# arneschneuing/DiffSBDD

Hardware: AMD Instinct MI355X
Metric: sampled ligands/sec (500-step DDPM, fullatom_cond) at 1/2/4/8 MI355X (higher is better)
Workload: dtype f32

## Files before the change

diffsbdd_amd/_lib.py:

```python
from __future__ import annotations

import ctypes as C
import os

_HERE = os.path.dirname(os.path.abspath(__file__))
LIB_PATH = os.environ.get("DSBDD_LIB") or os.path.join(_HERE, "libdiffsbdd_hip.so")
ABI_VERSION = 6

OK, ERR_ARG, ERR_STATE, ERR_CAPACITY, ERR_LAUNCH = 0, -1, -2, -3, -4
STATUS_NAN, STATUS_EDGE_OVERFLOW = 1, 2
MOL_MAX_ATOMS, MOL_STATS, FP_WORDS = 128, 8, 64

G_NAMES = ["ATOM_ENC_W0T", "ATOM_ENC_B0", "ATOM_ENC_W1T", "ATOM_ENC_B1",
           "RES_ENC_W0T", "RES_ENC_B0", "RES_ENC_W1T", "RES_ENC_B1",
           "ATOM_DEC_W0T", "ATOM_DEC_B0", "ATOM_DEC_W1T", "ATOM_DEC_B1",
           "RES_DEC_W0T", "RES_DEC_B0", "RES_DEC_W1T", "RES_DEC_B1",
           "EMB_WT", "EMB_B", "EMBOUT_WT", "EMBOUT_B"]
GCL_NAMES = ["E1_WT", "E1_WD", "E1_WD0", "E1_TAB", "E2_WT", "E2_B", "ATT_W", "ATT_B",
             "N1_WT", "N1_B", "N2_WT", "N2_B"]
EQ_NAMES = ["C1_WT", "C_WD", "C_WD0", "C_TAB", "C_W2T", "C_B2",
            "X_WD", "X_WD0", "X_TAB", "X_W2T", "X_B2", "W3"]
OPT_PRUNE, OPT_CONE, OPT_GRANULE16, OPT_EMU, OPT_SPLITK, OPT_SHELL, OPT_TAIL = 0, 1, 2, 3, 4, 5, 6
(BUF_EDGE_ROW, BUF_EDGE_COL, BUF_EDGE_D0, BUF_ROW_PTR, BUF_H, BUF_X, BUF_NODE_BATCH, BUF_DEG,
 BUF_LEVEL, BUF_LEVEL_LIST, BUF_LEVEL_COUNT, BUF_LEVEL_END, BUF_LROW_PTR, BUF_LEDGE_ROW, BUF_LEDGE_COL,
 BUF_LEDGE_D0, BUF_LEVEL_STATS) = range(17)


class Config(C.Structure):
    _fields_ = [(n, C.c_int32) for n in (
        "atom_nf", "residue_nf", "joint_nf", "hidden_nf", "n_layers", "inv_sublayers",
        "attention", "use_tanh", "update_pocket_coords", "reflection_equivariant",
        "edge_embedding_dim", "has_cutoff_ligand", "has_cutoff_pocket",
        "has_cutoff_interaction")] + [(n, C.c_float) for n in (
            "cutoff_ligand", "cutoff_pocket", "cutoff_interaction",
            "norm_constant", "normalization_factor", "coords_range")]


class TrainGraph(C.Structure):
    _fields_ = [(n, C.c_void_p) for n in ("erow", "ecol", "ed0", "row_ptr", "deg", "rev", "node_batch", "lig_off",
                                          "poc_off")] + [(n, C.c_int64) for n in ("n_lig", "n_nodes", "n_edges", "batch")]


class LossCfg(C.Structure):
    _fields_ = [(n, C.c_int32) for n in ("batch", "n_lig", "n_pocket", "atom_nf", "residue_nf", "timesteps", "remove_com",
                                         "vnode_idx")] + \
# ... 43 lines not shown
    "dsbdd_engine_set_option": (C.c_int, [_P, C.c_int, C.c_int]),
    "dsbdd_engine_get_option": (C.c_int, [_P, C.c_int]),
    "dsbdd_engine_profile": (C.c_int, [_P, C.c_int, C.c_int]),
    "dsbdd_engine_profile_read": (C.c_int, [_P, C.POINTER(C.c_double), C.POINTER(_I64)]),
    "dsbdd_cond_reverse_update": (C.c_int, [_P, _P, _P, _P, _P, _P, _P, _I64, _I64, _I64,
                                            _I32, _I32, _F, _F, _F, _I32]),
    "dsbdd_joint_reverse_update": (C.c_int, [_P, _P, _P, _P, _P, _P, _P, _P, _P, _I64, _I64, _I64,
                                             _I32, _I32, _F, _F, _F, _I32]),
    "dsbdd_segment_mean3": (C.c_int, [_P, _P, _I32, _P, _I64, _I64, _P]),
    "dsbdd_cond_affine_noise": (C.c_int, [_P, _P, _P, _P, _P, _P, _I64, _I64, _I64, _I32, _I32, _F, _F, _I32]),
    "dsbdd_joint_affine_noise": (C.c_int, [_P, _P, _P, _P, _P, _P, _P, _I64, _I64, _I64, _I32, _I32, _F, _F,
                                           _I32, _I32]),
    "dsbdd_cond_repaint_update": (C.c_int, [_P, _P, _P, _P, _P, _P, _P, _P, _P, _P, _P, _I64, _I64, _I64,
                                            _I32, _I32, _F, _F, _F, _F, _I32, _I32]),
    "dsbdd_joint_repaint_update": (C.c_int, [_P] * 15 + [_I64, _I64, _I64, _I32, _I32, _F, _F, _F, _F, _I32]),
    "dsbdd_cond_step_keyed": (C.c_int, [_P] * 10 + [_I64, _I64, _I64, _I32, _I32, _F, _F, _F, _I32, _F, _F, _F, _I32,
                                        C.c_uint64, C.c_uint64, _I64, _P, _P, _F]),
    "dsbdd_randn_keyed": (C.c_int, [_P, _P, _P, _I64, _I32, _I64, _I64, _P, C.c_uint64, C.c_uint64,
                                    C.c_uint32]),
    "dsbdd_node_linear": (C.c_int, [_P, _P, _I32, _I32, _P, _I32, _I32, _P, _I32, _P, _P, _I32,
                                    _P, _I32, _I64, _I32, _I32]),
    "dsbdd_chain_split_host": (_I64, [_I32, _I32, _I32, _P, _P, _P, _I32, _I32, _P, _P, _I64]),
    "dsbdd_chain_split_probe": (C.c_int, [_P, _I32, _P, _I32, _I32, _P, _P, _P, _I32, _I32, _P, _P, _I64, _P]),
    "dsbdd_build_edges": (C.c_int, [_P, _P, _P, _P, _I64, _I64, _I64, C.POINTER(Config),
                                    _P, _P, _P, _P, _P, _P, _P, _P, _I64, _P]),
    "dsbdd_bond_orders": (C.c_int, [_P, _P, _P, _P, _I64, _I32, _P, _P, _P, C.c_float, C.c_float,
                                    C.c_float, _I32, _P]),
    "dsbdd_mol_graph_stats": (C.c_int, [_P, _P, _P, _P, _I64, _I32, _P, _I32, _I32, _P, _P, _P, _P, _P, _P]),
    "dsbdd_fp_diversity": (C.c_int, [_P, _P, _P, _I64, _P, _P]),
    "dsbdd_pose_check": (C.c_int, [_P, _P, _P, _P, _I64, _P, _P, _P, _P, _I64, _F, _F, _P, _P]),
    "dsbdd_vina_type": (C.c_int, [_P, _P, _P, _P, _I64, _I32, _P, _I32, _P, _P]),
    "dsbdd_vina_score": (C.c_int, [_P, _P, _P, _P, _I64, _P, _P, _P, _P, _P, _I64, _P, _P, _P]),
    "dsbdd_vina_score_grad": (C.c_int, [_P, _P, _P, _P, _I64, _P, _P, _P, _P, _P, _I64, _P, _P, _P, _P, _P]),
    "dsbdd_vina_minimize": (C.c_int, [_P, _P, _P, _P, _I64, _P, _P, _P, _P, _P, _I64, _P, _P, _P, _P, _P, _F, _F, _I32, _P, _P,
                                      _P, _P]),
    "dsbdd_pack_ligands": (C.c_int, [_P, _P, _P, _P, _I32, _I64, _P, _P, _P, _I64, _I64, _I32, _P, _P, _P, _P, _P]),
    "dsbdd_train_scratch_bytes": (C.c_size_t, [_I32, _I64, _I64]),
    "dsbdd_train_wgrad_scratch_bytes": (C.c_size_t, [_I64, _I64, _I64]),
    "dsbdd_train_wgrad_plan_bytes": (C.c_size_t, [_I64, _I64, _I64]),
    "dsbdd_train_edge_rev": (C.c_int, [_P, _P, _P]),
    "dsbdd_train_sample_mean": (C.c_int, [_P, _P, _P, _P]),
    "dsbdd_train_gcl_forward": (C.c_int, [_P, _I32, _P, _P, _P, _F, _P, _P, C.c_size_t]),
    "dsbdd_train_gcl_backward": (C.c_int, [_P, _I32, _P, _P, _P, _F, _P, _P, _P, _P, C.c_size_t]),
    "dsbdd_train_coord_forward": (C.c_int, [_P, _I32, _P, _P, _I32, _P, _P, _I64, _F, _F, _I32, _F, _P, _P,
                                            C.c_size_t]),
    "dsbdd_train_coord_backward": (C.c_int, [_P, _I32, _P, _P, _I32, _P, _P, _I64, _I64, _F, _F, _I32, _F, _P, _P, _P,
# ... 91 lines not shown
```

diffsbdd_amd/csrc/capi_kernels.h:

```cpp
#pragma once

extern "C" {

int dsbdd_cond_reverse_update(void* stream, float* z_lig, float* xh_pocket, const float* eps_lig,
                              const float* noise, const int64_t* mask_lig, const int64_t* mask_pocket,
                              int64_t n_lig, int64_t n_pocket, int64_t batch, int32_t atom_nf,
                              int32_t residue_nf, float alpha_ts, float c_eps, float sigma, int32_t remove_com) {
  StreamDevice stream_device_(stream);
  if (!z_lig || !xh_pocket || !eps_lig || !noise || !mask_lig || !mask_pocket || batch < 1)
    return fail(DSBDD_ERR_ARG, "bad argument");
  hipLaunchKernelGGL(cond_update_kernel, dim3((int)batch), dim3(kThreads), 0, static_cast<hipStream_t>(stream),
                     z_lig, xh_pocket, eps_lig, noise, mask_lig, (int)n_lig, mask_pocket, (int)n_pocket,
                     3 + atom_nf, 3 + residue_nf, alpha_ts, c_eps, sigma, remove_com);
  HIP_TRY(hipGetLastError());
  return DSBDD_OK;
}

int dsbdd_joint_reverse_update(void* stream, float* z_lig, float* z_pocket, const float* eps_lig,
                               const float* eps_pocket, const float* noise_lig, const float* noise_pocket,
                               const int64_t* mask_lig, const int64_t* mask_pocket, int64_t n_lig,
                               int64_t n_pocket, int64_t batch, int32_t atom_nf, int32_t residue_nf,
                               float alpha_ts, float c_eps, float sigma, int32_t center_noise) {
  StreamDevice stream_device_(stream);
  if (!z_lig || !z_pocket || !eps_lig || !eps_pocket || !noise_lig || !noise_pocket || !mask_lig ||
// ... 122 lines not shown
  HIP_TRY(hipGetLastError());
  return DSBDD_OK;
}

int dsbdd_node_linear(void* stream, const float* A1, int32_t lda1, int32_t K1, const float* A2, int32_t lda2,
                      int32_t K2, const float* WT, int32_t ldw, const float* bias, const float* R, int32_t ldr,
                      float* C, int32_t ldc, int64_t M, int32_t N, int32_t act) {
  StreamDevice stream_device_(stream);
  if (!A1 || !WT || !C || K1 < 1 || K2 < 0 || (K2 > 0 && !A2) || (ldw & 3) || N > ldw ||
      (reinterpret_cast<uintptr_t>(WT) & 15))
    return fail(DSBDD_ERR_ARG, "bad argument (WT must be 16-byte aligned with ldw % 4 == 0)");
  HIP_TRY(nl(static_cast<hipStream_t>(stream), A1, lda1, K1, A2, lda2, K2, WT, ldw, bias, R, ldr, C, ldc, M, N, act));
  return DSBDD_OK;
}

static bool chain_split_args_ok(int32_t M, int32_t n_proj, const void* proj_N, const void* proj_first, const void* proj_count,
                                int32_t H, int32_t grid, const void* header, const void* pieces, int64_t capacity) {
  return header && capacity >= 0 && (capacity == 0 || pieces) && grid >= 1 && (H == 64 || H == 128 || H == 192 || H == 256) &&
         n_proj >= 0 && n_proj <= kChainMaxProj && (n_proj == 0 || (proj_N && proj_first && proj_count)) && M <= (8 << 20);
}
static const char* const kChainSplitBadArg =
    "bad argument (null output, grid < 1, H not 64 / 128 / 192 / 256, more than 3 projections or more than 8 M rows)";

int64_t dsbdd_chain_split_host(int32_t M, int32_t do_mlp, int32_t n_proj, const int32_t* proj_N,
                               const int32_t* proj_first, const int32_t* proj_count, int32_t H, int32_t grid,
                               uint32_t* header, int32_t* pieces, int64_t capacity) {
  if (!chain_split_args_ok(M, n_proj, proj_N, proj_first, proj_count, H, grid, header, pieces, capacity))
    return fail(DSBDD_ERR_ARG, kChainSplitBadArg);
  ChainSplitIn in{};
  in.M = M; in.do_mlp = do_mlp; in.n_proj = n_proj; in.H = H; in.grid = grid;
  for (int q = 0; q < n_proj; ++q) { in.N[q] = proj_N[q]; in.first[q] = proj_first[q]; in.count[q] = proj_count[q]; }
  const ChainSplit sp(in);
  sp.report(header);
  return chain_split_list(sp, grid, grid, ~0u, pieces, capacity);
}

int dsbdd_chain_split_probe(void* stream, int32_t M, const int32_t* m_count, int32_t do_mlp, int32_t n_proj,
                            const int32_t* proj_N, const int32_t* proj_first, const int32_t* const* proj_count,
                            int32_t H, int32_t grid, uint32_t* header, int32_t* pieces, int64_t capacity,
                            int64_t* n_pieces) {
  StreamDevice stream_device_(stream);
  if (!n_pieces || !chain_split_args_ok(M, n_proj, proj_N, proj_first, proj_count, H, grid, header, pieces, capacity))
    return fail(DSBDD_ERR_ARG, kChainSplitBadArg);
  NodeChainArgs a{};
  a.M = M; a.m_count = m_count; a.do_mlp = do_mlp; a.n_proj = n_proj;
  for (int q = 0; q < n_proj; ++q) { a.proj[q].N = proj_N[q]; a.proj[q].first = proj_first[q]; a.proj[q].count = proj_count[q]; }
  hipLaunchKernelGGL(chain_split_probe_kernel, dim3(grid), dim3(64), 0, static_cast<hipStream_t>(stream), a, (int)H, header,
                     pieces, (long long)capacity, reinterpret_cast<long long*>(n_pieces));
  HIP_TRY(hipGetLastError());
  return DSBDD_OK;
}

int dsbdd_bond_orders(void* stream, const float* x, const int32_t* atom_type, const int32_t* mol_off,
                      int64_t batch, int32_t n_types, const float* bonds1, const float* bonds2,
                      const float* bonds3, float margin1, float margin2, float margin3, int32_t n_max,
                      int8_t* order) {
  StreamDevice stream_device_(stream);
  if (!x || !atom_type || !mol_off || !bonds1 || !bonds2 || !bonds3 || !order || batch < 1 || n_types < 1 ||
      n_max < 1)
    return fail(DSBDD_ERR_ARG, "bad argument");
  hipStream_t s = static_cast<hipStream_t>(stream);
  HIP_TRY(hipMemsetAsync(order, 0, (size_t)batch * n_max * n_max, s));
  BondArgs a{x, atom_type, mol_off, bonds1, bonds2, bonds3, margin1, margin2, margin3, n_types, n_max,
             reinterpret_cast<signed char*>(order)};
  hipLaunchKernelGGL(bond_orders_kernel, dim3((unsigned)batch), dim3(64), 0, s, a);
  HIP_TRY(hipGetLastError());
  return DSBDD_OK;
}

int dsbdd_mol_graph_stats(void* stream, const int8_t* order, const int32_t* atom_type, const int32_t* mol_off, int64_t batch,
                          int32_t n_types, const int32_t* max_valence, int32_t n_max, int32_t orders_in_key,
                          int32_t* valence, int32_t* label, int32_t* stats, uint64_t* keys, uint32_t* fingerprint,
                          int32_t* type_counts) {
// ... 165 lines not shown
```

diffsbdd_amd/csrc/chain_split.h:

```cpp
#pragma once

#ifdef __HIPCC__
#define CHAIN_SPLIT_FN __host__ __device__ __forceinline__
#else
#define CHAIN_SPLIT_FN inline
#endif
namespace dsbdd {
constexpr int kChainRowsMax = 96;
constexpr int kChainMaxProj = 3;
constexpr int kChainAllRows = 0x7fffffff;
constexpr int kChainBreaks = 2 * kChainMaxProj + 3;
template <class T> CHAIN_SPLIT_FN T chain_min(T a, T b) { return b < a ? b : a; }
template <class T> CHAIN_SPLIT_FN T chain_max(T a, T b) { return a < b ? b : a; }
CHAIN_SPLIT_FN unsigned chain_share(unsigned a, unsigned j, unsigned n) { return a / n * j + (a % n * j + n - 1) / n; }

struct ChainSplitIn {
  int M;
  int do_mlp, n_proj;
  int N[kChainMaxProj];
  int first[kChainMaxProj];
  int count[kChainMaxProj];
  int H, grid;
};

// ... 129 lines not shown

  CHAIN_SPLIT_FN bool range(unsigned v, int& r0, int& r1) const {
    if (v >= Vs) return false;
    if (!forced) {
      r0 = v == 0 ? 0 : row_at(chain_share(total, v, V));
      r1 = v + 1 == V ? (Mw + 15) / 16 * 16 : row_at(chain_share(total, v + 1, V));
      return true;
    }
    unsigned j = v, ns = 1, f0 = 0, cseg = 0;
    int b0 = 0, b1 = Tt;
    bool found = false;
#pragma unroll
    for (int a2 = 0; a2 < kChainBreaks - 1; ++a2) {
      if (!found && j < nrg[a2]) { found = true; ns = nrg[a2]; f0 = fcut[a2]; cseg = fcut[a2 + 1] - fcut[a2]; b0 = cut[a2]; b1 = cut[a2 + 1]; }
      if (!found) j -= nrg[a2];
    }
    if (!found) return false;
    r0 = j == 0 ? (b0 << 4) : chain_min(chain_max(row_at(f0 + chain_share(cseg, j, ns)), b0 << 4), b1 << 4);
    r1 = j + 1 == ns ? (b1 << 4) : chain_min(chain_max(row_at(f0 + chain_share(cseg, j + 1, ns)), b0 << 4), b1 << 4);
    return true;
  }
};

template <class F>
CHAIN_SPLIT_FN void chain_pieces(int r0, int r1, F&& piece) {
  for (int nt = (r1 - r0) / 16, rs = r0; nt > 0;) {
    const int take = nt > kChainRowsMax / 16 ? kChainRowsMax / 16 : nt;
    piece(rs, take);
    rs += 16 * take; nt -= take;
  }
}

CHAIN_SPLIT_FN long long chain_split_list(const ChainSplit& sp, unsigned grid, unsigned wg_end, unsigned own, int* pieces,
                                          long long capacity) {
  long long n = 0;
  for (unsigned wg = 0; wg < wg_end; ++wg)
    for (unsigned v = wg; v < sp.Vs; v += grid) {
      int r0, r1;
      if (!sp.range(v, r0, r1)) break;
      chain_pieces(r0, r1, [&](int rs, int take) {
        if ((own == ~0u || own == wg) && n < capacity) { pieces[3 * n] = (int)wg; pieces[3 * n + 1] = rs; pieces[3 * n + 2] = take; }
        ++n;
      });
    }
  return n;
}

}
```

diffsbdd_amd/csrc/engine.hip:

```cpp
#include "../../include/diffsbdd_hip.h"

#include <algorithm>
#include <climits>
#include <cmath>
#include <cstdio>
#include <cstdlib>
#include <cstring>
#include <string>
#include <type_traits>
#include <utility>
#include <vector>

#include "common.h"
#include "ddpm.h"
#include "edge_mlp.h"
#include "edge_wave.h"
#include "edge_wave16.h"
#include "edge_splitk.h"
#include "graph_parts.h"
#include "radius_graph.h"
#include "level_list.h"
#include "geometry.h"
#include "lig_head.h"
#include "ligand_pack.h"
// ... 169 lines not shown
                           int32_t* n_stages, int32_t* timed_level) {
  if (!e || !radius || !ghost || !n_stages || !timed_level) return fail(DSBDD_ERR_ARG, "null argument");
  const int n = (int)e->plan_radius.size();
  if (capacity < n) return fail(DSBDD_ERR_CAPACITY, "plan arrays too short");
  for (int i = 0; i < n; ++i) { radius[i] = e->plan_radius[i]; ghost[i] = e->plan_ghost[i]; }
  *n_stages = n; *timed_level = e->plan_timed_level;
  return DSBDD_OK;
}

int dsbdd_engine_set_option(dsbdd_engine* e, int which, int value) {
  if (!e) return fail(DSBDD_ERR_ARG, "null argument");
  switch (which) {
    case DSBDD_OPT_PRUNE: e->prune = value ? 1 : 0; break;
    case DSBDD_OPT_CONE: e->cone = value <= 0 ? 0 : (value >= 2 ? 2 : 1); break;
    case DSBDD_OPT_GRANULE16: e->granule16 = (unsigned)value; break;
    case DSBDD_OPT_SPLITK: e->splitk = (unsigned)value; break;
    case DSBDD_OPT_EMU:
      if (value != 0 && value != 6 && value != 9) return fail(DSBDD_ERR_ARG, "DSBDD_OPT_EMU takes 0, 6 or 9");
      e->emu = value; break;
    case DSBDD_OPT_SHELL: e->shell = value ? 1 : 0; break;
    case DSBDD_OPT_TAIL:
      if (value < 0) return fail(DSBDD_ERR_ARG, "DSBDD_OPT_TAIL takes a value >= 0");
      e->tail = value; break;
    default: return fail(DSBDD_ERR_ARG, "unknown option");
  }
  e->drop_graphs();
  return DSBDD_OK;
}

int dsbdd_engine_get_option(const dsbdd_engine* e, int which) {
  if (!e) return fail(DSBDD_ERR_ARG, "null argument");
  switch (which) {
    case DSBDD_OPT_PRUNE: return e->prune;
    case DSBDD_OPT_CONE: return e->cone;
    case DSBDD_OPT_GRANULE16: return (int)e->granule16;
    case DSBDD_OPT_SPLITK: return (int)e->splitk;
    case DSBDD_OPT_EMU: return e->emu;
    case DSBDD_OPT_SHELL: return e->shell;
    case DSBDD_OPT_TAIL: return e->tail;
  }
  return fail(DSBDD_ERR_ARG, "unknown option");
}

int dsbdd_engine_set_trace(dsbdd_engine* e, float* th, float* tx) {
  if (!e) return DSBDD_ERR_ARG;
  e->trace_h = th; e->trace_x = tx;
  return DSBDD_OK;
}

int dsbdd_engine_profile(dsbdd_engine* e, int enable, int max_launches) {
  if (!e || max_launches < 0) return fail(DSBDD_ERR_ARG, "bad argument");
  e->profile = enable < 0 ? 0 : enable;
  e->prof_call = 0;
  e->ev_used = 0;
  while (e->profile && e->ev.size() < (size_t)2 * max_launches) {
    hipEvent_t a;
    HIP_TRY(hipEventCreate(&a));
    e->ev.push_back(a);
  }
  return DSBDD_OK;
}

// ... 96 lines not shown
```

diffsbdd_amd/csrc/engine_state.h:

```cpp
#pragma once

static thread_local std::string g_err;
static int fail(int code, const std::string& msg) { g_err = msg; return code; }

#define HIP_TRY(expr)                                                              \
  do {                                                                             \
    hipError_t _e = (expr);                                                        \
    if (_e != hipSuccess)                                                          \
      return fail(DSBDD_ERR_LAUNCH, std::string(#expr) + ": " + hipGetErrorString(_e)); \
  } while (0)
#define RC_TRY(expr)                       \
  do {                                     \
    const int _rc = (expr);                \
    if (_rc != DSBDD_OK) return _rc;       \
  } while (0)

struct StreamDevice {
  int prev = -1;
  bool switched = false;
  explicit StreamDevice(void* stream) {
    hipStream_t s = static_cast<hipStream_t>(stream);
    if (!s) return;
    hipDevice_t d = 0;
    int cur = 0;
// ... 103 lines not shown
  take(w.lvl, N); take(w.seg_rows, LB); take(w.seg_edges, LB);
  take(w.node_base, LB + 1); take(w.edge_base, LB + 1); take(w.lvl_cnt, 16); take(w.lvl_end, 16);
  take(w.lvl_list, NG); take(w.row_ptrL, NG + 1); take(w.erowL, EL); take(w.ecolL, EL); take(w.ed0L, EL);
  take(w.lvl_stats, 16); take(w.frame_rows, N);
  take(w.wchain, (size_t)c.n_layers * ((size_t)c.inv_sublayers * 5 * H * H + H * PQ) + 1024);
  w.total = off;
  return w;
}

struct dsbdd_engine : Workspace {
  dsbdd_config cfg;
  std::vector<const float*> slots;
  bool has_weights = false;
  char* ws = nullptr;
  size_t ws_bytes = 0;
  int64_t cap_lig = 0, cap_poc = 0, cap_batch = 0, cap_edges = 0;
  bool lvl_stats_zeroed = false;
  int64_t cap_edgesL = 0;
  int prune = 1;
  int cone = 1;
  int64_t ghost_slots = 0;
  int shell = 1;
  int tail = 1;
  int64_t cap_shell = 0;
  char* shell_mem = nullptr;
  int64_t shell_key[3] = {0, 0, 0};
  int *sh_seg = nullptr, *sh_deg = nullptr, *sh_ptr = nullptr, *sh_row = nullptr, *sh_col = nullptr, *sh_cnt = nullptr;
  float* sh_d0 = nullptr;
  unsigned long long* sh_stats = nullptr;
  float* msg_buf = nullptr;
  int64_t msg_cap = 0;
  std::vector<int> plan_radius, plan_ghost;
  int plan_timed_level = kLevels - 1;
  bool frame = false;
  int64_t frame_nlig = 0, frame_npoc = 0, frame_batch = 0, frame_n3 = 0, frame_cap3 = 0;
  bool ghost_dirty = true;
  bool h0_pocket_valid = false;
  int64_t cap_tiles = 0;
  int64_t cap_tiles16 = 0;
  unsigned granule16 = 0;
  unsigned splitk = 0;
  int emu = 0;
  DerivedReady derived;
  float *trace_h = nullptr, *trace_x = nullptr;
  int n_cu = 256;
  int chain = 1;
// ... 78 lines not shown
        kW2Kinds[kind].pack(s, src, w2_copy(e, kind, blk, which), c.hidden_nf);
        HIP_TRY(hipGetLastError());
      }
    e->derived.w2[kind] = true;
  }
  return DSBDD_OK;
}

static bool env_int(const char* name, long long* v, bool mask = false) {
  const char* s = getenv(name);
  if (!s) return false;
  *v = mask ? (long long)strtoul(s, nullptr, 0) : (long long)atoi(s);
  return true;
}
static int env_int_in(const char* name, long long lo, long long hi, int dflt) {
  long long v;
  return env_int(name, &v) && v >= lo && v <= hi ? (int)v : dflt;
}
static void read_env_switches(dsbdd_engine* e) {
  long long v;
  const std::pair<const char*, int*> off_on_zero[] = {
      {"DSBDD_GRAPH", &e->use_graph}, {"DSBDD_EDGE_BPERM", &e->edge_bperm}, {"DSBDD_COORD_SPLIT", &e->coord_split},
      {"DSBDD_NODE_GROUP", &e->node_group}, {"DSBDD_PRUNE", &e->prune}, {"DSBDD_LIG_HEAD", &e->lig_head},
      {"DSBDD_NODE_CHAIN", &e->chain}};
  for (const auto& sw : off_on_zero) if (env_int(sw.first, &v) && v == 0) *sw.second = 0;
  if (env_int("DSBDD_FOLD_SCAN", &v)) e->fold_scan = v > 0 ? 1 : 0;
  if (env_int("DSBDD_GRANULE16", &v, true)) e->granule16 = (unsigned)v;
  if (env_int("DSBDD_SPLITK", &v, true)) e->splitk = (unsigned)v;
  if (env_int("DSBDD_EMU", &v)) e->emu = (v == 6 || v == 9) ? (int)v : 0;
  if (env_int("DSBDD_CONE", &v)) e->cone = v <= 0 ? 0 : (v >= 2 ? 2 : 1);
  if (env_int("DSBDD_NODE_CHAIN_MIN_ROWS", &v) && v >= 0) e->chain_min_rows = v;
  if (env_int("DSBDD_EDGE_MAX_WG", &v) && v > 0) e->edge_max_wg = (int)v;
  if (env_int("DSBDD_TAIL", &v) && v >= 0) e->tail = (int)v;
}
```

diffsbdd_amd/csrc/forward.h:

```cpp
#pragma once

struct ForwardArgs {
  const float *xh_lig, *xh_pocket, *t;
  int64_t t_count;
  const int64_t *mask_lig, *mask_pocket;
  int64_t n_lig, n_pocket, batch;
  const int32_t *ext_row, *ext_col;
  int64_t ext_n_edges;
  float *eps_lig, *eps_pocket;
  int32_t* status;
};

static bool frame_applies(const dsbdd_engine* e, const ForwardArgs& a) {
  return e->frame && !e->cfg.update_pocket_coords && !a.ext_row && a.n_lig == e->frame_nlig &&
         a.n_pocket == e->frame_npoc && a.batch == e->frame_batch;
}

static Mlp2Problem residue_encoder(const dsbdd_engine* e, const ForwardArgs& a) {
  const dsbdd_config& c = e->cfg;
  const int r = c.residue_nf, J = c.joint_nf, JP = pad4(J + 1);
  const float* const* W = e->slots.data();
  return Mlp2Problem{a.xh_pocket + 3, 3 + r, r, W[DSBDD_G_RES_ENC_W0T], pad4(2 * r), W[DSBDD_G_RES_ENC_B0], 2 * r,
                     W[DSBDD_G_RES_ENC_W1T], pad4(J), W[DSBDD_G_RES_ENC_B1], J, e->h0 + (size_t)a.n_lig * JP, JP,
                     (int)a.n_pocket};
// ... 350 lines not shown
        const int QW = n_mlp * H;
        const float* wc = chain_w(blk, 0, 3);
        if (!subset) {
          ca.proj[ca.n_proj++] = ChainProj{wc, e->pq, PQ, PQ, nullptr, 0};
          st.chained_coord = true;
        } else if (prune && n1.row_idx) {
          ca.proj[ca.n_proj++] = ChainProj{wc, e->pq, PQ, QW, act_count, first};
          ca.proj[ca.n_proj++] = ChainProj{wc + (size_t)(QW / 16) * (H / 16) * 256, e->pq + QW, PQ, QW,
                                           e->lvl_cnt + kLevels, first};
          st.chained_coord = true;
        }
      }
      const bool has_next = !last_sub || blk + 1 < c.n_layers;
      if (has_next) {
        const int nb = last_sub ? blk + 1 : blk, ns = last_sub ? 0 : sub + 1;
        const NodeLinearArgs nx = gcl_pq(nb, ns);
        const bool same_rows = nx.row_idx == n1.row_idx && nx.m_count == n1.m_count && nx.M == n1.M;
        if (same_rows || ghost) {
          ca.proj[ca.n_proj++] = ChainProj{chain_w(nb, ns, 2), e->pqg, 2 * H, 2 * H, nullptr, 0};
          st.chained_pq = true;
          fill_pq = ghost && !same_rows;
        }
      }
      HIP_TRY(launch_node_chain(s, ca, H, e->n_cu));
    } else {
      HIP_TRY(launch_node_linear(s, n1));
      HIP_TRY(launch_node_linear(s, n2));
    }
    if (ghost) {
      const int hi = radius_of(g + 1) + 1 < LV ? radius_of(g + 1) + 1 : LV;
      if (hi > radius) {
        hipLaunchKernelGGL(canon_fill_kernel, dim3((N - nlig + 3) / 4), dim3(kThreads), 0, s, e->h,
                           (const int*)e->lvl, (const int*)e->twin, nlig, N, N, radius, hi, H,
                           fill_pq ? e->pqg : (float*)nullptr, 2 * H);
        HIP_TRY(hipGetLastError());
      }
    }
    return DSBDD_OK;
  }

  int coord_stage(int blk, StageState& st) {
    auto Q = [&](int which) { return W[eq_slot(c, blk, which)]; };
    const int QW = n_mlp * H;
    NodeLinearArgs grp[kMaxGroup];
    int ng = 0;
    if (!st.chained_coord) {
      if (subset) {
        grp[ng++] = NodeLinearArgs{e->h, H, H, nullptr, 0, 0, Q(DSBDD_EQ_C1_WT), PQ, nullptr, nullptr, 0, e->pq, PQ,
                                   (int)N, QW, 0, act_rows, act_count};
        grp[ng++] = NodeLinearArgs{e->h, H, H, nullptr, 0, 0, Q(DSBDD_EQ_C1_WT) + QW, PQ, nullptr, nullptr, 0,
                                   e->pq + QW, PQ, (int)n_lig, QW, 0, nullptr, nullptr};
      } else {
        grp[ng++] = NodeLinearArgs{e->h, H, H, nullptr, 0, 0, Q(DSBDD_EQ_C1_WT), PQ, nullptr, nullptr, 0, e->pq, PQ,
                                   (int)N, PQ, 0, nullptr, nullptr};
      }
    }
    const int n_coord = ng;
    const bool want_next = blk + 1 < c.n_layers && !st.chained_pq;
    if (st.chained_pq && blk + 1 < c.n_layers) st.pqg_ready = true;
    if (want_next && use_chain) {
      const NodeLinearArgs nx = gcl_pq(blk + 1, 0);
      NodeChainArgs ca{};
      ca.row_idx = nx.row_idx; ca.m_count = nx.m_count; ca.M = nx.M; ca.do_mlp = 0; ca.h = e->h;
      ca.n_proj = 1;
      ca.proj[0] = ChainProj{chain_w(blk + 1, 0, 2), e->pqg, 2 * H, 2 * H, nullptr, 0};
      HIP_TRY(launch_node_chain(s, ca, H, e->n_cu));
      st.pqg_ready = true;
    } else if (want_next) {
      grp[ng++] = gcl_pq(blk + 1, 0);
    }
    if (ng > 0) {
      if (e->node_group && launch_node_group(s, grp, ng) == hipSuccess) {
        if (ng > n_coord) st.pqg_ready = true;
      } else {
        (void)hipGetLastError();
        for (int i = 0; i < n_coord; ++i) HIP_TRY(launch_node_linear(s, grp[i]));
      }
    }
    st.chained_pq = false;
    const int S = c.inv_sublayers;
    EdgeArgs ea{};
    ea.erow = L_row + ghost_slots; ea.ecol = L_col + ghost_slots; ea.ed0 = L_d0 + ghost_slots; ea.e_count = e_upd;
    ea.e_cap = L_cap - (int)ghost_slots; ea.wt_base = (int)(ghost_slots / 32); ea.x = e->x;
    ea.n_lig = nlig; ea.n_nodes = N + n_frame_rows; ea.ldpq = PQ;
    ea.mlp[0] = edge_mlp(e->pq + QW, e->pq, Q(DSBDD_EQ_C_WD), Q(DSBDD_EQ_C_WD0), Q(DSBDD_EQ_C_TAB),
                         Q(DSBDD_EQ_C_W2T), Q(DSBDD_EQ_C_B2), blk, S);
    if (n_mlp == 2)
      ea.mlp[1] = edge_mlp(e->pq + QW + H, e->pq + H, Q(DSBDD_EQ_X_WD), Q(DSBDD_EQ_X_WD0), Q(DSBDD_EQ_X_TAB),
// ... 82 lines not shown
```

diffsbdd_amd/csrc/node_chain.h:

```cpp
#pragma once
#include "chain_split.h"
#include "common.h"

namespace dsbdd {

typedef float f32x4 __attribute__((ext_vector_type(4)));

#ifdef DSBDD_CHAIN_TS
__device__ unsigned long long* g_chain_ts = nullptr;
__device__ __forceinline__ void chain_ts(int slot) {
  if (g_chain_ts && threadIdx.x == 0 && slot < 16) {
    g_chain_ts[blockIdx.x * 32 + slot] = __builtin_readcyclecounter();
    g_chain_ts[blockIdx.x * 32 + 16 + slot] = wall_clock64();
  }
}
#define CHAIN_TS(k) chain_ts(k)
#define CHAIN_NOTE(slot, v) do { if (g_chain_ts && threadIdx.x == 0) g_chain_ts[blockIdx.x * 32 + (slot)] = (unsigned long long)(v); } while (0)
#else
#define CHAIN_TS(k) do { } while (0)
#define CHAIN_NOTE(slot, v) do { } while (0)
#endif

constexpr int kChainThreads = 512;
constexpr int kChainChunkK = 64;
// ... 5 lines not shown
  const int g = rest % (K / 16), ct = rest / (K / 16);
  dst[idx] = WT[(size_t)(16 * g + 4 * (lane >> 4) + s) * ldw + 16 * ct + (lane & 15)];
}

struct ChainProj {
  const float* Wp;
  float* C; int ldc;
  int N;
  const int* count;
  int first;
};

struct NodeChainArgs {
  const int* row_idx;
  const int* m_count;
  int M;
  int do_mlp;
  float* h;
  const float* agg;
  const float* W1p; const float* b1;
  const float* W2p; const float* b2;
  int n_proj;
  ChainProj proj[kChainMaxProj];
};

__device__ __forceinline__ f32x4 mfma16(float a, float b, f32x4 c) {
  return __builtin_amdgcn_mfma_f32_16x16x4f32(a, b, c, 0, 0, 0);
}

template <int RT, int CT>
__device__ __forceinline__ void chain_mfma_group(f32x4 (&acc)[RT][CT], const float4 (&wv)[CT], const float4 (&xv)[RT]) {
  __builtin_amdgcn_s_setprio(1);
#pragma unroll
  for (int s = 0; s < 4; ++s)
#pragma unroll
    for (int rt = 0; rt < RT; ++rt)
#pragma unroll
      for (int t = 0; t < CT; ++t) {
        const float a = s == 0 ? wv[t].x : (s == 1 ? wv[t].y : (s == 2 ? wv[t].z : wv[t].w));
        const float b = s == 0 ? xv[rt].x : (s == 1 ? xv[rt].y : (s == 2 ? xv[rt].z : xv[rt].w));
        acc[rt][t] = mfma16(a, b, acc[rt][t]);
      }
  __builtin_amdgcn_s_setprio(0);
}

template <int RT, int CT, bool CHUNKED, class XOf, class Hook>
// ... 212 lines not shown
  CHAIN_TS(7);
}

__device__ __forceinline__ ChainSplitIn chain_split_input(const NodeChainArgs& p, int H, int grid) {
  ChainSplitIn in{};
  in.M = p.m_count ? min(p.M, *p.m_count) : p.M;
  in.do_mlp = p.do_mlp; in.n_proj = p.n_proj; in.H = H; in.grid = grid;
  if (in.M <= 0) return in;
#pragma unroll
  for (int q = 0; q < kChainMaxProj; ++q)
    if (q < p.n_proj) {
      in.N[q] = p.proj[q].N; in.first[q] = p.proj[q].first;
      in.count[q] = p.proj[q].count ? *p.proj[q].count : kChainAllRows;
    }
  return in;
}

template <int H>
__global__ __launch_bounds__(kChainThreads, 2) void node_chain_kernel(NodeChainArgs p) {
  __shared__ float smem[kChainRowsMax * H + 2 * (kChainChunkK / 4) * kChainRowsMax * 4];
  CHAIN_TS(0);
  const ChainSplitIn in = chain_split_input(p, H, (int)gridDim.x);
  CHAIN_NOTE(11, (unsigned long long)(in.M > 0 ? wall_clock64() : 0));
  const ChainSplit sp(in);
  const int cnt[kChainMaxProj] = {sp.cnt[0], sp.cnt[1], sp.cnt[2]};
  for (unsigned v = blockIdx.x; v < sp.Vs; v += gridDim.x) {
    int r0, r1;
    if (!sp.range(v, r0, r1)) break;
    CHAIN_NOTE(12, (unsigned long long)(r1 >= r0 ? wall_clock64() : 0));
    chain_pieces(r0, r1, [&](int rs, int take) {
      switch (take) {
        case 1: chain_range<H, 1>(p, rs, sp.Mw, smem, cnt); break;
        case 2: chain_range<H, 2>(p, rs, sp.Mw, smem, cnt); break;
        case 3: chain_range<H, 3>(p, rs, sp.Mw, smem, cnt); break;
        case 4: chain_range<H, 4>(p, rs, sp.Mw, smem, cnt); break;
        case 5: chain_range<H, 5>(p, rs, sp.Mw, smem, cnt); break;
        default: chain_range<H, 6>(p, rs, sp.Mw, smem, cnt); break;
      }
    });
  }
}

__global__ void chain_split_probe_kernel(NodeChainArgs p, int H, unsigned* header, int* pieces, long long capacity,
                                         long long* n_pieces) {
  if (threadIdx.x != 0) return;
  const ChainSplit sp(chain_split_input(p, H, (int)gridDim.x));
  const long long n = chain_split_list(sp, gridDim.x, blockIdx.x + 1, blockIdx.x, pieces, capacity);
  if (blockIdx.x == gridDim.x - 1) { sp.report(header); *n_pieces = n; }
}

inline hipError_t launch_node_chain(hipStream_t s, const NodeChainArgs& a, int H, int n_cu) {
  if (a.M <= 0) return hipSuccess;
  if (a.M > (8 << 20)) return hipErrorInvalidValue;
  dim3 grid(n_cu), block(kChainThreads);
  switch (H) {
    case 256: hipLaunchKernelGGL((node_chain_kernel<256>), grid, block, 0, s, a); break;
    case 192: hipLaunchKernelGGL((node_chain_kernel<192>), grid, block, 0, s, a); break;
    case 128: hipLaunchKernelGGL((node_chain_kernel<128>), grid, block, 0, s, a); break;
    case 64: hipLaunchKernelGGL((node_chain_kernel<64>), grid, block, 0, s, a); break;
    default: return hipErrorInvalidValue;
  }
  return hipGetLastError();
}

}
```

include/diffsbdd_hip.h:

```cpp
#ifndef DIFFSBDD_HIP_H
#define DIFFSBDD_HIP_H

#include <stddef.h>
#include <stdint.h>

#ifdef __cplusplus
extern "C" {
#endif

#define DSBDD_ABI_VERSION 6

enum {
  DSBDD_OK = 0,
  DSBDD_ERR_ARG = -1,
  DSBDD_ERR_STATE = -2,
  DSBDD_ERR_CAPACITY = -3,
  DSBDD_ERR_LAUNCH = -4
};

enum {
  DSBDD_STATUS_NAN = 1,
  DSBDD_STATUS_EDGE_OVERFLOW = 2
};

// ... 62 lines not shown
                                  const int32_t* frame_rows, const int32_t* twin_local, int64_t n_lig,
                                  int64_t n_pocket, int64_t batch, int64_t n_frame, int64_t batch_frame,
                                  int64_t edge_bound_frame);
int dsbdd_engine_clear_pocket_frame(dsbdd_engine* e);

int dsbdd_engine_set_trace(dsbdd_engine* e, float* trace_h, float* trace_x);

int dsbdd_dynamics_forward(dsbdd_engine* e, void* stream, const float* xh_lig,
                           const float* xh_pocket, const float* t, int64_t t_count,
                           const int64_t* mask_lig, const int64_t* mask_pocket, int64_t n_lig,
                           int64_t n_pocket, int64_t batch, const int32_t* ext_row,
                           const int32_t* ext_col, int64_t ext_n_edges, float* eps_lig,
                           float* eps_pocket, int32_t* status);

int dsbdd_engine_profile(dsbdd_engine* e, int enable, int max_launches);
int dsbdd_engine_profile_read(dsbdd_engine* e, double* total_ms, int64_t* launches);

int dsbdd_engine_graph_stats(const dsbdd_engine* e, int64_t* replays, int64_t* captures, int64_t* eager);

int dsbdd_engine_last_plan(const dsbdd_engine* e, int32_t* radius, int32_t* ghost, int32_t capacity,
                           int32_t* n_stages, int32_t* timed_level);

enum { DSBDD_OPT_PRUNE = 0, DSBDD_OPT_CONE = 1, DSBDD_OPT_GRANULE16 = 2, DSBDD_OPT_EMU = 3, DSBDD_OPT_SPLITK = 4,
       DSBDD_OPT_SHELL = 5, DSBDD_OPT_TAIL = 6 };
int dsbdd_engine_set_option(dsbdd_engine* e, int which, int value);
int dsbdd_engine_get_option(const dsbdd_engine* e, int which);

enum {
  DSBDD_BUF_EDGE_ROW = 0, DSBDD_BUF_EDGE_COL, DSBDD_BUF_EDGE_D0, DSBDD_BUF_ROW_PTR,
  DSBDD_BUF_H, DSBDD_BUF_X, DSBDD_BUF_NODE_BATCH, DSBDD_BUF_DEG,
  DSBDD_BUF_LEVEL, DSBDD_BUF_LEVEL_LIST, DSBDD_BUF_LEVEL_COUNT, DSBDD_BUF_LEVEL_END,
  DSBDD_BUF_LROW_PTR, DSBDD_BUF_LEDGE_ROW, DSBDD_BUF_LEDGE_COL, DSBDD_BUF_LEDGE_D0,
  DSBDD_BUF_LEVEL_STATS
};
int dsbdd_engine_buffer(const dsbdd_engine* e, int which, void** ptr_out);

enum { DSBDD_SHELL_STATS = 0, DSBDD_SHELL_COUNT, DSBDD_SHELL_ROW, DSBDD_SHELL_COL, DSBDD_SHELL_PTR, DSBDD_SHELL_DEG };
int dsbdd_engine_shell_read(const dsbdd_engine* e, int which, int list, void* dst, int64_t count);

enum { DSBDD_LIST2_DEG = 0, DSBDD_LIST2_ROW_PTR };
int dsbdd_engine_list2_read(const dsbdd_engine* e, int which, void* dst, int64_t count);

int dsbdd_cond_reverse_update(void* stream, float* z_lig, float* xh_pocket, const float* eps_lig,
                              const float* noise, const int64_t* mask_lig,
                              const int64_t* mask_pocket, int64_t n_lig, int64_t n_pocket,
                              int64_t batch, int32_t atom_nf, int32_t residue_nf, float alpha_ts,
                              float c_eps, float sigma, int32_t remove_com);
// ... 40 lines not shown
                               const float* noise_jump_pocket, const int64_t* mask_lig,
                               const int64_t* mask_pocket, int64_t n_lig, int64_t n_pocket, int64_t batch,
                               int32_t atom_nf, int32_t residue_nf, float alpha_s, float sigma_s,
                               float alpha_ts, float sigma_ts, int32_t jump);

int dsbdd_randn_keyed(void* stream, float* out, const int64_t* mask, int64_t n_rows,
                      int32_t n_cols, int64_t batch, int64_t sample_offset,
                      const int64_t* sample_ids, uint64_t seed, uint64_t draw_index,
                      uint32_t stream_id);

int dsbdd_node_linear(void* stream, const float* A1, int32_t lda1, int32_t K1, const float* A2,
                      int32_t lda2, int32_t K2, const float* WT, int32_t ldw, const float* bias,
                      const float* R, int32_t ldr, float* C, int32_t ldc, int64_t M, int32_t N,
                      int32_t act);

int64_t dsbdd_chain_split_host(int32_t M, int32_t do_mlp, int32_t n_proj, const int32_t* proj_N,
                               const int32_t* proj_first, const int32_t* proj_count, int32_t H, int32_t grid,
                               uint32_t* header, int32_t* pieces, int64_t capacity);

int dsbdd_chain_split_probe(void* stream, int32_t M, const int32_t* m_count, int32_t do_mlp, int32_t n_proj,
                            const int32_t* proj_N, const int32_t* proj_first, const int32_t* const* proj_count,
                            int32_t H, int32_t grid, uint32_t* header, int32_t* pieces, int64_t capacity,
                            int64_t* n_pieces);

int dsbdd_build_edges(void* stream, const float* x, const int64_t* mask_lig,
                      const int64_t* mask_pocket, int64_t n_lig, int64_t n_pocket, int64_t batch,
                      const dsbdd_config* cfg, int32_t* node_batch, int32_t* lig_off,
                      int32_t* poc_off, int32_t* deg, int32_t* row_ptr, int32_t* edge_row,
                      int32_t* edge_col, float* edge_d0, int64_t edge_capacity, int32_t* status);

typedef struct dsbdd_train_graph {
  const int32_t *erow, *ecol; const float* ed0;
  const int32_t *row_ptr, *deg;
  const int32_t* rev;
  const int32_t *node_batch, *lig_off, *poc_off;
  int64_t n_lig, n_nodes, n_edges, batch;
} dsbdd_train_graph;

typedef struct dsbdd_train_mlp {
  const float *P, *Q; int32_t ldpq;
  const float *wd, *wd0, *tab;
  const float *W2, *W2T, *b2;
  const float *head, *head_b;
} dsbdd_train_mlp;

typedef struct dsbdd_train_mlp_grad {
// ... 190 lines not shown
```

Measured before the change: 42.36.

## Add weighted segment-dealing work split for node chain kernel, enabled by default

Introduces a ChainDeal scheduler that cuts the row-tile range at projection boundaries into segments, weights each by its per-tile cost, and packs contiguous tile runs so each workgroup's load is balanced under a bound found by iterative relaxation. The node-chain kernel uses this dealing by default and falls back to the old ChainSplit when there are too many segments relative to the grid. The aim is less load imbalance and tail idleness across CUs in the fused node MLP/projection chain. In exchange, every block computes the plan on device, and the loop past the first range moves in single 16-row tiles, which could change how many pieces each block handles.

```diff
diff --git a/diffsbdd_amd/_lib.py b/diffsbdd_amd/_lib.py
--- a/diffsbdd_amd/_lib.py
+++ b/diffsbdd_amd/_lib.py
@@ -20,7 +20,7 @@
              "N1_WT", "N1_B", "N2_WT", "N2_B"]
 EQ_NAMES = ["C1_WT", "C_WD", "C_WD0", "C_TAB", "C_W2T", "C_B2",
             "X_WD", "X_WD0", "X_TAB", "X_W2T", "X_B2", "W3"]
-OPT_PRUNE, OPT_CONE, OPT_GRANULE16, OPT_EMU, OPT_SPLITK, OPT_SHELL, OPT_TAIL = 0, 1, 2, 3, 4, 5, 6
+OPT_PRUNE, OPT_CONE, OPT_GRANULE16, OPT_EMU, OPT_SPLITK, OPT_SHELL, OPT_TAIL, OPT_CHAIN_DEAL = 0, 1, 2, 3, 4, 5, 6, 7
 (BUF_EDGE_ROW, BUF_EDGE_COL, BUF_EDGE_D0, BUF_ROW_PTR, BUF_H, BUF_X, BUF_NODE_BATCH, BUF_DEG,
  BUF_LEVEL, BUF_LEVEL_LIST, BUF_LEVEL_COUNT, BUF_LEVEL_END, BUF_LROW_PTR, BUF_LEDGE_ROW, BUF_LEDGE_COL,
  BUF_LEDGE_D0, BUF_LEVEL_STATS) = range(17)
@@ -110,6 +110,8 @@
                                     _P, _I32, _I64, _I32, _I32]),
     "dsbdd_chain_split_host": (_I64, [_I32, _I32, _I32, _P, _P, _P, _I32, _I32, _P, _P, _I64]),
     "dsbdd_chain_split_probe": (C.c_int, [_P, _I32, _P, _I32, _I32, _P, _P, _P, _I32, _I32, _P, _P, _I64, _P]),
+    "dsbdd_chain_deal_host": (_I64, [_I32, _I32, _I32, _P, _P, _P, _I32, _I32, _P, _P, _I64]),
+    "dsbdd_chain_deal_probe": (C.c_int, [_P, _I32, _P, _I32, _I32, _P, _P, _P, _I32, _I32, _P, _P, _I64, _P]),
     "dsbdd_build_edges": (C.c_int, [_P, _P, _P, _P, _I64, _I64, _I64, C.POINTER(Config),
                                     _P, _P, _P, _P, _P, _P, _P, _P, _I64, _P]),
     "dsbdd_bond_orders": (C.c_int, [_P, _P, _P, _P, _I64, _I32, _P, _P, _P, C.c_float, C.c_float,
diff --git a/diffsbdd_amd/csrc/capi_kernels.h b/diffsbdd_amd/csrc/capi_kernels.h
--- a/diffsbdd_amd/csrc/capi_kernels.h
+++ b/diffsbdd_amd/csrc/capi_kernels.h
@@ -168,33 +168,64 @@
 static const char* const kChainSplitBadArg =
     "bad argument (null output, grid < 1, H not 64 / 128 / 192 / 256, more than 3 projections or more than 8 M rows)";
 
-int64_t dsbdd_chain_split_host(int32_t M, int32_t do_mlp, int32_t n_proj, const int32_t* proj_N,
-                               const int32_t* proj_first, const int32_t* proj_count, int32_t H, int32_t grid,
-                               uint32_t* header, int32_t* pieces, int64_t capacity) {
+extern "C++" {
+template <class Split>
+static int64_t chain_split_host(int32_t M, int32_t do_mlp, int32_t n_proj, const int32_t* proj_N, const int32_t* proj_first,
+                                const int32_t* proj_count, int32_t H, int32_t grid, uint32_t* header, int32_t* pieces,
+                                int64_t capacity) {
   if (!chain_split_args_ok(M, n_proj, proj_N, proj_first, proj_count, H, grid, header, pieces, capacity))
     return fail(DSBDD_ERR_ARG, kChainSplitBadArg);
   ChainSplitIn in{};
   in.M = M; in.do_mlp = do_mlp; in.n_proj = n_proj; in.H = H; in.grid = grid;
   for (int q = 0; q < n_proj; ++q) { in.N[q] = proj_N[q]; in.first[q] = proj_first[q]; in.count[q] = proj_count[q]; }
-  const ChainSplit sp(in);
+  const Split sp(in);
   sp.report(header);
   return chain_split_list(sp, grid, grid, ~0u, pieces, capacity);
 }
 
-int dsbdd_chain_split_probe(void* stream, int32_t M, const int32_t* m_count, int32_t do_mlp, int32_t n_proj,
-                            const int32_t* proj_N, const int32_t* proj_first, const int32_t* const* proj_count,
-                            int32_t H, int32_t grid, uint32_t* header, int32_t* pieces, int64_t capacity,
-                            int64_t* n_pieces) {
+template <class Split>
+static int chain_split_probe(void* stream, int32_t M, const int32_t* m_count, int32_t do_mlp, int32_t n_proj,
+                             const int32_t* proj_N, const int32_t* proj_first, const int32_t* const* proj_count, int32_t H,
+                             int32_t grid, uint32_t* header, int32_t* pieces, int64_t capacity, int64_t* n_pieces) {
   StreamDevice stream_device_(stream);
   if (!n_pieces || !chain_split_args_ok(M, n_proj, proj_N, proj_first, proj_count, H, grid, header, pieces, capacity))
     return fail(DSBDD_ERR_ARG, kChainSplitBadArg);
   NodeChainArgs a{};
   a.M = M; a.m_count = m_count; a.do_mlp = do_mlp; a.n_proj = n_proj;
   for (int q = 0; q < n_proj; ++q) { a.proj[q].N = proj_N[q]; a.proj[q].first = proj_first[q]; a.proj[q].count = proj_count[q]; }
-  hipLaunchKernelGGL(chain_split_probe_kernel, dim3(grid), dim3(64), 0, static_cast<hipStream_t>(stream), a, (int)H, header,
-                     pieces, (long long)capacity, reinterpret_cast<long long*>(n_pieces));
-  HIP_TRY(hipGetLastError());
-  return DSBDD_OK;
+  hipLaunchKernelGGL(chain_split_probe_kernel<Split>, dim3(grid), dim3(64), 0, static_cast<hipStream_t>(stream), a, (int)H,
+                     header, pieces, (long long)capacity, reinterpret_cast<long long*>(n_pieces));
+  HIP_TRY(hipGetLastError());
+  return DSBDD_OK;
+}
+}
+
+int64_t dsbdd_chain_split_host(int32_t M, int32_t do_mlp, int32_t n_proj, const int32_t* proj_N,
+                               const int32_t* proj_first, const int32_t* proj_count, int32_t H, int32_t grid,
+                               uint32_t* header, int32_t* pieces, int64_t capacity) {
+  return chain_split_host<ChainSplit>(M, do_mlp, n_proj, proj_N, proj_first, proj_count, H, grid, header, pieces, capacity);
+}
+
+int dsbdd_chain_split_probe(void* stream, int32_t M, const int32_t* m_count, int32_t do_mlp, int32_t n_proj,
+                            const int32_t* proj_N, const int32_t* proj_first, const int32_t* const* proj_count,
+                            int32_t H, int32_t grid, uint32_t* header, int32_t* pieces, int64_t capacity,
+                            int64_t* n_pieces) {
+  return chain_split_probe<ChainSplit>(stream, M, m_count, do_mlp, n_proj, proj_N, proj_first, proj_count, H, grid, header,
+                                       pieces, capacity, n_pieces);
+}
+
+int64_t dsbdd_chain_deal_host(int32_t M, int32_t do_mlp, int32_t n_proj, const int32_t* proj_N,
+                              const int32_t* proj_first, const int32_t* proj_count, int32_t H, int32_t grid,
+                              uint32_t* header, int32_t* pieces, int64_t capacity) {
+  return chain_split_host<ChainDealt>(M, do_mlp, n_proj, proj_N, proj_first, proj_count, H, grid, header, pieces, capacity);
+}
+
+int dsbdd_chain_deal_probe(void* stream, int32_t M, const int32_t* m_count, int32_t do_mlp, int32_t n_proj,
+                           const int32_t* proj_N, const int32_t* proj_first, const int32_t* const* proj_count,
+                           int32_t H, int32_t grid, uint32_t* header, int32_t* pieces, int64_t capacity,
+                           int64_t* n_pieces) {
+  return chain_split_probe<ChainDealt>(stream, M, m_count, do_mlp, n_proj, proj_N, proj_first, proj_count, H, grid, header,
+                                      pieces, capacity, n_pieces);
 }
 
 int dsbdd_bond_orders(void* stream, const float* x, const int32_t* atom_type, const int32_t* mol_off,
diff --git a/diffsbdd_amd/csrc/chain_split.h b/diffsbdd_amd/csrc/chain_split.h
--- a/diffsbdd_amd/csrc/chain_split.h
+++ b/diffsbdd_amd/csrc/chain_split.h
@@ -175,6 +175,143 @@
   }
 };
 
+constexpr int kDealCuts = 2 * kChainMaxProj + 2;
+constexpr int kChainSegs = kDealCuts - 1;
+
+struct ChainDeal {
+  int cnt[kChainMaxProj];
+  int Mw, Tt;
+  int cut[kDealCuts];
+  unsigned k[kChainSegs];
+  unsigned nrg[kChainSegs];
+  unsigned B;
+  unsigned Vs;
+  bool fallback;
+
+  CHAIN_SPLIT_FN explicit ChainDeal(const ChainSplitIn& in) {
+    Mw = 0; Tt = 0; B = 0; Vs = 0; fallback = false;
+#pragma unroll
+    for (int q = 0; q < kChainMaxProj; ++q) cnt[q] = 0;
+    const int M = in.M;
+    if (M <= 0) return;
+    const unsigned w_mlp = in.do_mlp ? 48u : 0u;
+    int M_work = in.do_mlp ? M : 0;
+    bool work = in.do_mlp != 0;
+    unsigned wgt[kChainMaxProj];
+    int lo[kChainMaxProj];
+#pragma unroll
+    for (int q = 0; q < kChainMaxProj; ++q) {
+      const bool on = q < in.n_proj;
+      lo[q] = on ? chain_max(in.first[q], 0) : 0;
+      const int fst = chain_min(M, lo[q]);
+      cnt[q] = on ? chain_max(chain_min(M - fst, in.count[q]), 0) : 0;
+      wgt[q] = on ? (unsigned)(in.N[q] * 16 / in.H) : 0u;
+      M_work = chain_max(M_work, fst + cnt[q]);
+      work = work || (wgt[q] > 0 && cnt[q] > 0);
+    }
+    if (M_work <= 0 || !work) return;
+    Mw = M_work;
+    Tt = (Mw + 15) >> 4;
+    int t0[kChainMaxProj], t1[kChainMaxProj];
+#pragma unroll
+    for (int q = 0; q < kChainMaxProj; ++q) {
+      const int l = chain_min(lo[q], Tt << 4);
+      t0[q] = chain_min(Tt, l >> 4);
+      t1[q] = chain_min(Tt, (l + cnt[q] + 15) >> 4);
+    }
+    {
+      int nb = 0;
+      cut[nb++] = 0;
+#pragma unroll
+      for (int q = 0; q < kChainMaxProj; ++q) { cut[nb++] = t0[q]; cut[nb++] = t1[q]; }
+      cut[nb++] = Tt;
+#pragma unroll
+      for (int a2 = 1; a2 < kDealCuts; ++a2)
+#pragma unroll
+        for (int b2 = kDealCuts - 1; b2 > 0; --b2)
+          if (b2 <= a2 && cut[b2] < cut[b2 - 1]) { const int tmp = cut[b2]; cut[b2] = cut[b2 - 1]; cut[b2 - 1] = tmp; }
+    }
+    unsigned u[kChainSegs], S = 0, total = 0, u_max = 0;
+#pragma unroll
+    for (int a2 = 0; a2 < kChainSegs; ++a2) {
+      const unsigned T = (unsigned)(cut[a2 + 1] - cut[a2]);
+      unsigned c = w_mlp;
+#pragma unroll
+      for (int q = 0; q < kChainMaxProj; ++q) c += cut[a2] >= t0[q] && cut[a2] < t1[q] ? wgt[q] : 0u;
+      u[a2] = c; k[a2] = 1; nrg[a2] = T;
+      S += T > 0; total += T * c;
+      if (T > 0) u_max = chain_max(u_max, c);
+    }
+    const unsigned G = (unsigned)in.grid;
+    fallback = 8 * S > G && (unsigned)Tt >= 3 * G;
+    if (fallback) return;
+    if ((unsigned)Tt <= G || S > G) { Vs = (unsigned)Tt; B = 16 * u_max; return; }
+    unsigned b = chain_max(u_max, (total + G - 1) / G);
+    Vs = 0;
+#pragma unroll
+    for (int a2 = 0; a2 < kChainSegs; ++a2) {
+      const unsigned T = (unsigned)(cut[a2 + 1] - cut[a2]);
+      if (T > 0) {
+        k[a2] = u[a2] > 0 ? chain_min(b / u[a2], T) : T;
+        nrg[a2] = (T + k[a2] - 1) / k[a2];
+        Vs += nrg[a2];
+      }
+    }
+#pragma unroll 1
+    while (Vs > G) {
+      unsigned nb = ~0u;
+#pragma unroll
+      for (int a2 = 0; a2 < kChainSegs; ++a2)
+        if (k[a2] < (unsigned)(cut[a2 + 1] - cut[a2])) nb = chain_min(nb, (k[a2] + 1) * u[a2]);
+      b = nb;
+#pragma unroll
+      for (int a2 = 0; a2 < kChainSegs; ++a2) {
+        const unsigned T = (unsigned)(cut[a2 + 1] - cut[a2]);
+        if (k[a2] < T && (k[a2] + 1) * u[a2] == b) {
+          Vs -= nrg[a2];
+          k[a2] += 1;
+          nrg[a2] = (T + k[a2] - 1) / k[a2];
+          Vs += nrg[a2];
+        }
+      }
+    }
+    (void)b;
+#pragma unroll
+    for (int a2 = 0; a2 < kChainSegs; ++a2)
+      if (cut[a2 + 1] > cut[a2]) B = chain_max(B, 16 * u[a2] * chain_min(k[a2], (unsigned)(cut[a2 + 1] - cut[a2])));
+  }
+
+
+  CHAIN_SPLIT_FN bool range(unsigned v, int& r0, int& r1) const {
+    if (v >= Vs) return false;
+    unsigned j = v, kk = 1;
+    int b0 = 0, b1 = 0;
+    bool found = false;
+#pragma unroll
+    for (int a2 = 0; a2 < kChainSegs; ++a2) {
+      if (!found && j < nrg[a2]) { found = true; kk = k[a2]; b0 = cut[a2]; b1 = cut[a2 + 1]; }
+      if (!found) j -= nrg[a2];
+    }
+    if (!found) return false;
+    r0 = (b0 + (int)(j * kk)) << 4;
+    r1 = chain_min(b1, b0 + (int)((j + 1) * kk)) << 4;
+    return true;
+  }
+};
+
+struct ChainDealt {
+  ChainDeal dl;
+  ChainSplit sp;
+  unsigned Vs, grid;
+  CHAIN_SPLIT_FN explicit ChainDealt(const ChainSplitIn& in) : dl(in), sp(dl.fallback ? in : ChainSplitIn{}) {
+    Vs = dl.fallback ? sp.Vs : dl.Vs; grid = (unsigned)in.grid;
+  }
+  CHAIN_SPLIT_FN bool range(unsigned v, int& r0, int& r1) const { return dl.fallback ? sp.range(v, r0, r1) : dl.range(v, r0, r1); }
+  CHAIN_SPLIT_FN void report(unsigned* h) const {
+    h[0] = (unsigned)dl.Mw; h[1] = dl.B; h[2] = dl.Mw > 0 ? grid : 0u; h[3] = Vs; h[4] = dl.fallback;
+  }
+};
+
 template <class F>
 CHAIN_SPLIT_FN void chain_pieces(int r0, int r1, F&& piece) {
   for (int nt = (r1 - r0) / 16, rs = r0; nt > 0;) {
@@ -184,7 +321,8 @@
   }
 }
 
-CHAIN_SPLIT_FN long long chain_split_list(const ChainSplit& sp, unsigned grid, unsigned wg_end, unsigned own, int* pieces,
+template <class Split>
+CHAIN_SPLIT_FN long long chain_split_list(const Split& sp, unsigned grid, unsigned wg_end, unsigned own, int* pieces,
                                           long long capacity) {
   long long n = 0;
   for (unsigned wg = 0; wg < wg_end; ++wg)
diff --git a/diffsbdd_amd/csrc/engine.hip b/diffsbdd_amd/csrc/engine.hip
--- a/diffsbdd_amd/csrc/engine.hip
+++ b/diffsbdd_amd/csrc/engine.hip
@@ -215,6 +215,7 @@
     case DSBDD_OPT_TAIL:
       if (value < 0) return fail(DSBDD_ERR_ARG, "DSBDD_OPT_TAIL takes a value >= 0");
       e->tail = value; break;
+    case DSBDD_OPT_CHAIN_DEAL: e->chain_deal = value ? 1 : 0; break;
     default: return fail(DSBDD_ERR_ARG, "unknown option");
   }
   e->drop_graphs();
@@ -231,6 +232,7 @@
     case DSBDD_OPT_EMU: return e->emu;
     case DSBDD_OPT_SHELL: return e->shell;
     case DSBDD_OPT_TAIL: return e->tail;
+    case DSBDD_OPT_CHAIN_DEAL: return e->chain_deal;
   }
   return fail(DSBDD_ERR_ARG, "unknown option");
 }
diff --git a/diffsbdd_amd/csrc/engine_state.h b/diffsbdd_amd/csrc/engine_state.h
--- a/diffsbdd_amd/csrc/engine_state.h
+++ b/diffsbdd_amd/csrc/engine_state.h
@@ -149,6 +149,7 @@
   int64_t ghost_slots = 0;
   int shell = 1;
   int tail = 1;
+  int chain_deal = 1;
   int64_t cap_shell = 0;
   char* shell_mem = nullptr;
   int64_t shell_key[3] = {0, 0, 0};
@@ -273,7 +274,7 @@
   const std::pair<const char*, int*> off_on_zero[] = {
       {"DSBDD_GRAPH", &e->use_graph}, {"DSBDD_EDGE_BPERM", &e->edge_bperm}, {"DSBDD_COORD_SPLIT", &e->coord_split},
       {"DSBDD_NODE_GROUP", &e->node_group}, {"DSBDD_PRUNE", &e->prune}, {"DSBDD_LIG_HEAD", &e->lig_head},
-      {"DSBDD_NODE_CHAIN", &e->chain}};
+      {"DSBDD_NODE_CHAIN", &e->chain}, {"DSBDD_CHAIN_DEAL", &e->chain_deal}};
   for (const auto& sw : off_on_zero) if (env_int(sw.first, &v) && v == 0) *sw.second = 0;
   if (env_int("DSBDD_FOLD_SCAN", &v)) e->fold_scan = v > 0 ? 1 : 0;
   if (env_int("DSBDD_GRANULE16", &v, true)) e->granule16 = (unsigned)v;
diff --git a/diffsbdd_amd/csrc/forward.h b/diffsbdd_amd/csrc/forward.h
--- a/diffsbdd_amd/csrc/forward.h
+++ b/diffsbdd_amd/csrc/forward.h
@@ -396,6 +396,7 @@
           fill_pq = ghost && !same_rows;
         }
       }
+      ca.deal = e->chain_deal;
       HIP_TRY(launch_node_chain(s, ca, H, e->n_cu));
     } else {
       HIP_TRY(launch_node_linear(s, n1));
@@ -438,6 +439,7 @@
       ca.row_idx = nx.row_idx; ca.m_count = nx.m_count; ca.M = nx.M; ca.do_mlp = 0; ca.h = e->h;
       ca.n_proj = 1;
       ca.proj[0] = ChainProj{chain_w(blk + 1, 0, 2), e->pqg, 2 * H, 2 * H, nullptr, 0};
+      ca.deal = e->chain_deal;
       HIP_TRY(launch_node_chain(s, ca, H, e->n_cu));
       st.pqg_ready = true;
     } else if (want_next) {
diff --git a/diffsbdd_amd/csrc/node_chain.h b/diffsbdd_amd/csrc/node_chain.h
--- a/diffsbdd_amd/csrc/node_chain.h
+++ b/diffsbdd_amd/csrc/node_chain.h
@@ -51,6 +51,7 @@
   const float* W2p; const float* b2;
   int n_proj;
   ChainProj proj[kChainMaxProj];
+  int deal;
 };
 
 __device__ __forceinline__ f32x4 mfma16(float a, float b, f32x4 c) {
@@ -309,29 +310,52 @@
   CHAIN_TS(0);
   const ChainSplitIn in = chain_split_input(p, H, (int)gridDim.x);
   CHAIN_NOTE(11, (unsigned long long)(in.M > 0 ? wall_clock64() : 0));
-  const ChainSplit sp(in);
-  const int cnt[kChainMaxProj] = {sp.cnt[0], sp.cnt[1], sp.cnt[2]};
-  for (unsigned v = blockIdx.x; v < sp.Vs; v += gridDim.x) {
-    int r0, r1;
-    if (!sp.range(v, r0, r1)) break;
+  bool split = p.deal == 0;
+  unsigned Vs = 0;
+  int Mw = 0, first_r0 = 0, first_r1 = 0;
+  int cnt[kChainMaxProj] = {0, 0, 0};
+  if (!split) {
+    const ChainDeal dl(in);
+    split = dl.fallback;
+    if (!split) {
+      Vs = dl.Vs; Mw = dl.Mw;
+#pragma unroll
+      for (int q = 0; q < kChainMaxProj; ++q) cnt[q] = dl.cnt[q];
+      if (!dl.range(blockIdx.x, first_r0, first_r1)) Vs = 0;
+    }
+  }
+  const ChainSplit sp(split ? in : ChainSplitIn{});
+  if (split) {
+    Vs = sp.Vs; Mw = sp.Mw;
+#pragma unroll
+    for (int q = 0; q < kChainMaxProj; ++q) cnt[q] = sp.cnt[q];
+  }
+  for (unsigned v = blockIdx.x; v < Vs; v += gridDim.x) {
+    int r0 = first_r0, r1 = first_r1;
+    if (split) {
+      if (!sp.range(v, r0, r1)) break;
+    } else if (v != blockIdx.x) {
+      r0 = (int)v << 4; r1 = r0 + 16;
+    }
     CHAIN_NOTE(12, (unsigned long long)(r1 >= r0 ? wall_clock64() : 0));
     chain_pieces(r0, r1, [&](int rs, int take) {
       switch (take) {
-        case 1: chain_range<H, 1>(p, rs, sp.Mw, smem, cnt); break;
-        case 2: chain_range<H, 2>(p, rs, sp.Mw, smem, cnt); break;
-        case 3: chain_range<H, 3>(p, rs, sp.Mw, smem, cnt); break;
-        case 4: chain_range<H, 4>(p, rs, sp.Mw, smem, cnt); break;
-        case 5: chain_range<H, 5>(p, rs, sp.Mw, smem, cnt); break;
-        default: chain_range<H, 6>(p, rs, sp.Mw, smem, cnt); break;
+        case 1: chain_range<H, 1>(p, rs, Mw, smem, cnt); break;
+        case 2: chain_range<H, 2>(p, rs, Mw, smem, cnt); break;
+        case 3: chain_range<H, 3>(p, rs, Mw, smem, cnt); break;
+        case 4: chain_range<H, 4>(p, rs, Mw, smem, cnt); break;
+        case 5: chain_range<H, 5>(p, rs, Mw, smem, cnt); break;
+        default: chain_range<H, 6>(p, rs, Mw, smem, cnt); break;
       }
     });
   }
 }
 
+template <class Split>
 __global__ void chain_split_probe_kernel(NodeChainArgs p, int H, unsigned* header, int* pieces, long long capacity,
                                          long long* n_pieces) {
   if (threadIdx.x != 0) return;
-  const ChainSplit sp(chain_split_input(p, H, (int)gridDim.x));
+  const Split sp(chain_split_input(p, H, (int)gridDim.x));
   const long long n = chain_split_list(sp, gridDim.x, blockIdx.x + 1, blockIdx.x, pieces, capacity);
   if (blockIdx.x == gridDim.x - 1) { sp.report(header); *n_pieces = n; }
 }
diff --git a/include/diffsbdd_hip.h b/include/diffsbdd_hip.h
--- a/include/diffsbdd_hip.h
+++ b/include/diffsbdd_hip.h
@@ -108,7 +108,7 @@
                            int32_t* n_stages, int32_t* timed_level);
 
 enum { DSBDD_OPT_PRUNE = 0, DSBDD_OPT_CONE = 1, DSBDD_OPT_GRANULE16 = 2, DSBDD_OPT_EMU = 3, DSBDD_OPT_SPLITK = 4,
-       DSBDD_OPT_SHELL = 5, DSBDD_OPT_TAIL = 6 };
+       DSBDD_OPT_SHELL = 5, DSBDD_OPT_TAIL = 6, DSBDD_OPT_CHAIN_DEAL = 7 };
 int dsbdd_engine_set_option(dsbdd_engine* e, int which, int value);
 int dsbdd_engine_get_option(const dsbdd_engine* e, int which);
 
@@ -195,6 +195,14 @@
                             const int32_t* proj_N, const int32_t* proj_first, const int32_t* const* proj_count,
                             int32_t H, int32_t grid, uint32_t* header, int32_t* pieces, int64_t capacity,
                             int64_t* n_pieces);
+
+int64_t dsbdd_chain_deal_host(int32_t M, int32_t do_mlp, int32_t n_proj, const int32_t* proj_N,
+                              const int32_t* proj_first, const int32_t* proj_count, int32_t H, int32_t grid,
+                              uint32_t* header, int32_t* pieces, int64_t capacity);
+int dsbdd_chain_deal_probe(void* stream, int32_t M, const int32_t* m_count, int32_t do_mlp, int32_t n_proj,
+                           const int32_t* proj_N, const int32_t* proj_first, const int32_t* const* proj_count,
+                           int32_t H, int32_t grid, uint32_t* header, int32_t* pieces, int64_t capacity,
+                           int64_t* n_pieces);
 
 int dsbdd_build_edges(void* stream, const float* x, const int64_t* mask_lig,
                       const int64_t* mask_pocket, int64_t n_lig, int64_t n_pocket, int64_t batch,
```

New measurement: 43.57, median of 6. 2.9% higher.
